# thanosDelatolas/eva-vos

Hardware: AMD Instinct MI355X
Metric: frames/sec STCN mask-propagate 480p 1-obj (higher is better)
Workload: dtype f32; 1 GPU; DAVIS-17-val-shaped 480x854 (padded 480x864) single-object STCN propagate: fresh engine, interact(mask,0), T=66 frames/video, mem_freq=5, top_k=50; one video per step per GPU; videos_per_gpu=38, streams_per_gpu=4, key_lookahead=0, clips=8 distinct synthetic clips (one per pooled engine), weights=synthetic recipe seed 0 (no checkpoints offline)

## Files before the change

eva_vos_amd/_lib.py:

```python
from __future__ import annotations

import ctypes as C
import os

import torch

_HERE = os.path.dirname(os.path.abspath(__file__))
LIB_PATH = os.environ.get("STCN_LIB") or os.path.join(_HERE, "libstcn_hip.so")

K_CLASSES = ("conv", "conv_reduce", "memread", "elementwise", "conv_n1", "other", "wino_input", "fusion_conv", "attention")


class WeightDesc(C.Structure):
    _fields_ = [("name", C.c_char_p), ("data", C.c_void_p), ("ndim", C.c_int32), ("shape", C.c_int64 * 4)]


class EngineOpts(C.Structure):
    _fields_ = [(n, C.c_int32) for n in ("lookahead", "decode_batch", "key_batch", "fuse_side")]


class ModelOpts(C.Structure):
    _fields_ = [("top_k", C.c_int32), ("km", C.c_float)]


# ... 22 lines not shown
    "stcn_test_transpose": (_I, [_P, _P, _P, _I, _I, _I, _L, _L, _I]),
    "stcn_engine_create": (_I, [_P, _I, _I, _I, _I, _I, _P, _P, _P, _P, C.POINTER(_P)]),
    "stcn_engine_create_ex": (_I, [_P, _I, _I, _I, _I, _I, _P, _P, _P, _P, C.POINTER(EngineOpts), C.POINTER(_P)]),
    "stcn_engine_get_opts": (_I, [_P, C.POINTER(EngineOpts)]),
    "stcn_engine_destroy": (_I, [_P]),
    "stcn_engine_reset": (_I, [_P]),
    "stcn_engine_clone": (_I, [_P, _P, _P, _P, C.POINTER(_P)]),
    "stcn_interact": (_I, [_P, _P, _I, _I, _I]),
    "stcn_get_stats": (_I, [_P, C.POINTER(Stats)]),
    "stcn_get_flops": (_I, [_P, C.POINTER(_D)]),
    "stcn_last_conv_path": (C.c_char_p, []),
    "stcn_test_conv_trace": (_I, [_I]),
    "stcn_test_conv_trace_get": (C.c_char_p, []),
    "stcn_test_conv": (_I, [_P, _P, _P, _P, _P, _P] + [_I] * 11),
    "stcn_test_conv_ex": (_I, [_P, _P, _P, _P, _P, _P] + [_I] * 11 + [_P, _I, _L, _L, _L, _I, _L]),
    "stcn_test_conv_path": (_I, [_I] * 9 + [C.c_char_p, _I]),
    "stcn_test_conv_plan": (_I, [_I] * 9 + [C.POINTER(C.c_int32), _I, C.POINTER(_D)]),
    "stcn_test_sweep_plan": (_I, [_I, _I, _I, _I, C.POINTER(C.c_int32), _I, C.POINTER(C.c_int32)]),
    "stcn_test_encode_key": (_I, [_P, _P, _P, _I, _I, _P, _P, _P, _P, _P]),
    "stcn_test_encode_value": (_I, [_P, _P, _P, _P, _P, _I, _I, _I, _P]),
    "stcn_test_memory_read": (_I, [_P, _P, _P, _P, _I, _I, _I, _P, _P, _P]),
    "stcn_test_memory_read_k": (_I, [_P, _P, _P, _P, _I, _I, _I, _I, _P, _P, _P]),
    "stcn_test_memory_read_km": (_I, [_P, _P, _P, _P, _I, _I, _I, _I, _I, _I, _F, _P, _P, _P, _P]),
    "stcn_bench_memory_read": (_I, [_P, _P, _P, _P, _I, _I, _I, _I, _P, C.POINTER(_F), C.POINTER(C.c_int32)]),
    "stcn_bench_memory_read_k": (_I, [_P, _P, _P, _P, _I, _I, _I, _I, _I, _P, C.POINTER(_F), C.POINTER(C.c_int32)]),
    "stcn_bench_memory_read_km": (_I, [_P, _P, _P, _P, _I, _I, _I, _I, _I, _I, _F, _I, _P, C.POINTER(_F), C.POINTER(C.c_int32)]),
    "stcn_memread_plan": (_I, [_I, _I, C.POINTER(C.c_int32)]),
    "stcn_memread_scratch": (_I, [_I, C.POINTER(C.c_int64)]),
    "stcn_test_kernel": (_I, [C.c_char_p, _P, C.POINTER(_P), _I, C.POINTER(C.c_int64), _I, C.POINTER(_D), _I]),
    "stcn_test_fail_at": (_I, [_I]),
    "stcn_test_side_delay_us": (_I, [_I]),
    "stcn_test_decode": (_I, [_P, _P, _P, _P, _P, _P, _I, _I, _I, _P, _P]),
    "stcn_test_attention": (_I, [_P, _P, _P, _P, _P, _I, _I, _I, _P]),
    "stcn_test_fusion": (_I, [_P, _P, _P, _P, _P, _P, _F, _F, _I, _I, _P]),
# ... 59 lines not shown
```

eva_vos_amd/csrc/conv_gemm.hip:

```cpp
#include <hip/hip_ext.h>

#include <cstdio>
#include <cstdlib>
#include <mutex>
#include <set>
#include <type_traits>
#include <utility>

#include "kernels.h"

namespace stcn {

typedef float f32x4 __attribute__((ext_vector_type(4)));
typedef float f32x16 __attribute__((ext_vector_type(16)));

static constexpr int BK = 32;
static constexpr int LDT = 36;

typedef unsigned u32x4 __attribute__((ext_vector_type(4)));
static constexpr unsigned OOB = 0x80000000u;

struct TileDiv { FastDiv ntile, tiles_n, per_panel; int tiles_m; };
__device__ __forceinline__ void tile_to_mn(int tile, int tiles_n, int ntile, int pn, const TileDiv &td, int &tm, int &tn) {
    if (pn > 0 && tiles_n % pn == 0 && tiles_n > pn) {
// ... 495 lines not shown
                __builtin_amdgcn_sched_barrier(0);
            }
        }
        __syncthreads();
        if (--k_left == 0) { k_left = nkt; tile_end(); }
    };
    const int total = ((tile1 - tile0 + tstep - 1) / tstep) * nkt;
    int it = 0;
    for (; it + 1 < total; it += 2) {
        step(I0{});
        step(I1{});
    }
    if (it < total) step(I0{});
}

static int pw_chain_tiles(const ConvP &p, int force_splitk) {
    if (!p.kn.pw_chain || force_splitk > 0 || !p.pointwise || !p.affine_out || p.N <= 32 || (p.Cin % 32) != 0) return 0;
    if ((p.N % 64) != 0 && ((long)p.M + 64) * p.N * 4 >= (1L << 31)) return 0;
    const long ntile = (long)((p.M + 63) / 64) * ((p.N + 63) / 64);
    const long resident = (long)device_cus() * STCN_PW_WAVES;
    if (ntile < resident + resident / 2) return 0;
    const long nt = (ntile + resident - 1) / resident;
    return (int)(nt > 16 ? 16 : nt);
}

__global__ __launch_bounds__(256) void conv_reduce_kernel(const ConvP p) {
    const long total4 = (long)p.M * p.N / 4;
    const int ohw = p.OH * p.OW;
    const long slab = (long)p.M * p.N;
    for (long i = blockIdx.x * 256L + threadIdx.x; i < total4; i += (long)gridDim.x * 256) {
// ... 99 lines not shown

void conv_plan(ConvP &p, int force_splitk, size_t ws_floats, ConvPlan &cp) {
    static const int big_mode = env_int("STCN_CONV_BIG", 1);
    Plan pl = plan_variant(p, false, force_splitk, ws_floats);
    constexpr int big_mink = 2304;
    const bool big_ok = big_mode != 0 && !narrow_variant(p) && !smallc_variant(p) && p.N >= 128 && p.Kp >= big_mink;
    if (big_ok) {
        const Plan pb = plan_variant(p, true, force_splitk, ws_floats);
        if (pb.cost < pl.cost || big_mode >= 2) pl = pb;
    }
    p.panel = 4;
    p.tile_big = pl.big; p.splitk = pl.splitk;
    p.rem_full = pl.rem_full; p.rem_split = pl.rem_split; p.rem_per = pl.rem_per;
    p.chain = pw_chain_tiles(p, force_splitk);
    if (p.chain) { p.tile_big = 0; p.splitk = 1; p.rem_full = p.rem_split = p.rem_per = 0; }
    static const bool dbg = getenv("STCN_CONV_PLAN_DEBUG") != nullptr;
    if (dbg)
        fprintf(stderr, "conv_plan M=%d N=%d K=%d: %s splitk=%d tail=(%d full, %d pieces of %d) cost %.0f\n", p.M, p.N, p.Kp,
                pl.big ? "128x128" : (narrow_variant(p) ? "128x32" : "64x64"), pl.splitk, pl.rem_full, pl.rem_split, pl.rem_per, pl.cost);
    cp.family = CONV_DIRECT;
    cp.variant = conv_variant_name(p);
    cp.splitk = p.splitk; cp.tail = p.rem_split > 1;
    cp.n_in = 0; cp.n_gemm = 1; cp.reduce = p.splitk > 1 || p.rem_split > 1;
    cp.fl_exec = cp.fl;
}

int device_cus() {
    static const int cus = [] { int dev = 0, n = 256; (void)hipGetDevice(&dev); (void)hipDeviceGetAttribute(&n, hipDeviceAttributeMultiprocessorCount, dev); return n > 0 ? n : 256; }();
    return cus;
}

void allow_big_lds(const void *kernel, size_t lds) {
    if (lds <= 64 * 1024) return;
    static std::mutex mu;
    static std::set<std::pair<int, const void *>> done;
    int dev = 0;
// ... 4 lines not shown
}

void conv_launch(const ConvP &p, hipStream_t s, hipEvent_t *ev_gemm, hipEvent_t *ev_red) {
    const bool narrow = narrow_variant(p), big = p.tile_big != 0;
    const int BM = narrow ? 128 : (big ? 128 : 64), BN = narrow ? 32 : (big ? 128 : 64);
    const int tiles_m = (p.M + BM - 1) / BM, tiles_n = (p.N + BN - 1) / BN;
    const int ntile = tiles_m * tiles_n;
    const int nkt = p.Kp / BK;
    const int per = (nkt + p.splitk - 1) / p.splitk;
    const size_t lds = (size_t)2 * (BM + BN) * LDT * sizeof(float);
    const bool tail = p.rem_split > 1;
    const dim3 grid(tail ? p.rem_full + (ntile - p.rem_full) * p.rem_split : ntile * p.splitk);
    const bool smallc = smallc_variant(p);
    const int pn = p.panel;
    const TileDiv td{fastdiv_make((unsigned)ntile), fastdiv_make((unsigned)tiles_n), fastdiv_make((unsigned)(tiles_m * (pn > 0 ? pn : 1))), tiles_m};
    if (p.chain) {
        const dim3 cgrid((unsigned)((ntile + p.chain - 1) / p.chain));
        launch(p.relu_in ? pw_chain_kernel<true> : pw_chain_kernel<false>, cgrid, dim3(256), lds, s, ev_gemm, p, tiles_n, ntile, p.chain, td);
        return;
    }
#define STCN_INST(WM_, WN_, RM_, RN_, SC_, RL_, ...) kfn = conv_gemm_kernel<WM_, WN_, RM_, RN_, SC_, RL_, ##__VA_ARGS__>
    auto STCN_INST(2, 2, 1, 1, false, false);
    const bool pw = p.pointwise && !big && !narrow && !smallc;
    const int key = (pw ? 16 : 0) | (big ? 8 : 0) | (narrow ? 4 : 0) | (smallc ? 2 : 0) | (p.relu_in ? 1 : 0);
    switch (key) {
        case 16: STCN_INST(2, 2, 1, 1, false, false, true); break;
        case 17: STCN_INST(2, 2, 1, 1, false, true, true); break;
        case 0: break;
        case 1: STCN_INST(2, 2, 1, 1, false, true); break;
        case 2: STCN_INST(2, 2, 1, 1, true, false); break;
// ... 147 lines not shown
```

eva_vos_amd/csrc/engine.cpp:

```cpp
#include "engine.h"
#include "src_hash.h"

#include <algorithm>
#include <atomic>
#include <cmath>
#include <cstdarg>
#include <cstdio>
#include <cstdlib>
#include <cstring>
#include <map>
#include <mutex>
#include <unordered_map>
#include <utility>

namespace stcn {

static thread_local char g_err[512] = "";
void set_error(const char *fmt, ...) {
    va_list ap;
    va_start(ap, fmt);
    vsnprintf(g_err, sizeof(g_err), fmt, ap);
    va_end(ap);
}
const char *get_error() { return g_err; }

Knobs Knobs::from_env() {
    Knobs k;
    k.wino_min_cin = env_int("STCN_WINO_MIN_CIN", k.wino_min_cin);
    k.wino_ppw = env_int("STCN_WINO_PPW", k.wino_ppw);
    k.wino4_chunk_mb = env_int("STCN_WINO4_CHUNK_MB", k.wino4_chunk_mb);
    k.fusion_conv12 = env_int("STCN_FUSION_CONV12", k.fusion_conv12) != 0;
    k.fusion_wino = env_int("STCN_FUSION_WINO", k.fusion_wino) != 0;
    k.pw_chain = env_int("STCN_PW_CHAIN", k.pw_chain);
    return k;
}

void Prof::reset() {
    for (int i = 0; i < STCN_K_COUNT; ++i) { flops[i] = 0; bytes[i] = 0; exec_flops[i] = 0; launches[i] = 0; }
    hbm_conv_flops = hbm_conv_bytes = hbm_conv_ms = 0; hbm_conv_launches = 0;
    wino2_flops = wino4_flops = 0;
    for (auto &e : events) { pool.push_back(e.a); pool.push_back(e.b); }
    events.clear();
}
Prof::Ev &Prof::push_pair(int cls, bool hbm) {
    Ev e; e.cls = cls; e.hbm = hbm;
    for (hipEvent_t *p : {&e.a, &e.b}) {
        if (!pool.empty()) { *p = pool.back(); pool.pop_back(); }
        else (void)hipEventCreate(p);
// ... 447 lines not shown
    p.relu_in = a.relu_in; p.relu_out = a.relu_out;
    p.fd_ohw = fastdiv_make((unsigned)(p.OH * p.OW));
    p.fd_ow = fastdiv_make((unsigned)p.OW);
    p.fd_cin = fastdiv_make((unsigned)p.Cin);
    p.fd_kw = fastdiv_make((unsigned)p.KW);
    p.pointwise = cw.kh == 1 && cw.kw == 1 && a.stride == 1 && !a.x1 && bs0 == (long)H * W * c0;
    p.affine_out = (a.y_bs == 0 || a.y_bs == (long)p.OH * p.OW * p.N) && (!a.res || (res_bs == (long)p.OH * p.OW * p.N && !a.res_bmod)) &&
                   ((long)p.M + 128) * p.N * 4 < (1L << 32);
    p.partial = w.splitk;
    p.kn = w.kn;
    pl = ConvPlan{};
    pl.fl = 2.0 * p.M * p.N * (double)(cw.kh * cw.kw * cw.cin);
    if (a.force_splitk <= 0 && (fusion_conv_plan(p, pl) || wino4_plan(p, m.wino4_min_wg, w.wino_v_floats, w.splitk_floats, pl) ||
                                wino_plan(p, w.wino_v_floats, w.splitk_floats, pl)))
        return STCN_OK;
    conv_plan(p, a.force_splitk, w.splitk_floats, pl);
    return STCN_OK;
}

int run_conv(const Model &m, Work &w, hipStream_t s, const std::string &name, const ConvArgs &a) {
    ConvP p;
    ConvPlan &pl = g_path.plan;
    const int rc = plan_conv(m, w, name, a, p, pl);
    if (rc) return rc;
    hipEvent_t *eg[W4_MAX_CHUNKS] = {}, *ei[W4_MAX_CHUNKS] = {}, *er = nullptr;
    if (w.prof) {
        const double in0 = (double)(p.bs0 ? p.B : 1) * p.H * p.W * p.c0, in1 = p.x1 ? (double)(p.bs1 ? p.B : 1) * p.H * p.W * p.c1 : 0.0;
        const double resb = p.res ? (p.res_bs ? (double)p.M * p.N : (double)p.OH * p.OW * p.N) : 0.0;
        const double bytes = 4.0 * (in0 + in1 + (double)p.N * p.K + (double)p.M * p.N + resb);
        const bool hbm_bound = pl.fl / bytes < 157.3e12 / 8.0e12;
        const int cls = w.conv_cls;
        const bool hbm_acc = hbm_bound && cls == STCN_K_CONV;
        w.prof->bytes[cls] += bytes;
        w.prof->flops[cls] += pl.fl;
        w.prof->exec_flops[cls] += pl.fl_exec;
        if (hbm_acc) { w.prof->hbm_conv_bytes += bytes; w.prof->hbm_conv_flops += pl.fl; }
        if (pl.family == CONV_WINO4) w.prof->wino4_flops += pl.fl; else if (pl.family == CONV_WINO2) w.prof->wino2_flops += pl.fl;
        for (int c = 0; c < pl.n_gemm; ++c) {
            eg[c] = w.prof->attach(cls, hbm_acc);
            if (c < pl.n_in) ei[c] = w.prof->attach(STCN_K_WINO_INPUT);
        }
        if (pl.reduce) er = w.prof->attach(STCN_K_CONV_REDUCE);
    }
    if (g_trace_on) { char b[96]; g_trace += name; g_trace += '='; g_trace += format_conv_path(pl, b, sizeof(b)); g_trace += '\n'; }
    switch (pl.family) {
    case CONV_FUSION: fusion_conv_launch(p, pl, s, eg[0]); break;
    case CONV_WINO4: wino4_launch(p, pl, w.wino_v, s, ei, eg, er); break;
    case CONV_WINO2: wino_launch(p, pl, w.wino_v, s, ei[0], eg[0], er); break;
    default: conv_launch(p, s, eg[0], er);
    }
    return launch_status(name.c_str());
}

#define RC(x) do { int rc_ = (x); if (rc_) return rc_; } while (0)

int encode_key(const Model &m, Work &w, hipStream_t s, const float *img4, const KeyOut &o, int B, long out_bs) {
    const Dims &d = w.d;
    const long obs = B > 1 ? out_bs : 0;
    const long ibs = obs ? obs : CONV_DENSE;
    RC(run_conv(m, w, s, "key_encoder.conv1", ConvArgs(img4, 4, B, d.nh, d.nw).strided(2).out(w.A).relu(0, 1)));
    { Scope sc(w.prof, STCN_K_ELEMWISE, s); maxpool3x3s2_launch(w.A, w.B, B, d.h2, d.w2, 64, s); }
    struct St { const char *name; int n, planes, stride; } stages[3] = {{"res2", 3, 64, 1}, {"layer2", 4, 128, 2}, {"layer3", 6, 256, 2}};
    int H = d.h4, W = d.w4, cin = 64;
    float *x = w.B;
    for (int si = 0; si < 3; ++si) {
        const St &st = stages[si];
        for (int i = 0; i < st.n; ++i) {
            const std::string p = std::string("key_encoder.") + st.name + "." + std::to_string(i);
            const int sd = i == 0 ? st.stride : 1;
            const int OH = H / sd, OW = W / sd;
            const float *idt = x;
            if (i == 0) { RC(run_conv(m, w, s, p + ".downsample.0", ConvArgs(x, cin, B, H, W).strided(sd).out(w.D))); idt = w.D; }
            RC(run_conv(m, w, s, p + ".conv1", ConvArgs(x, cin, B, H, W).out(w.C).relu(0, 1)));
            RC(run_conv(m, w, s, p + ".conv2", ConvArgs(w.C, st.planes, B, H, W).strided(sd).out(w.A).relu(0, 1)));
            float *dst = x;
            long dst_bs = 0;
            if (si == 2 && i == st.n - 1) { dst = o.f16; dst_bs = obs; }
            RC(run_conv(m, w, s, p + ".conv3", ConvArgs(w.A, st.planes, B, OH, OW).out(dst, dst_bs).residual(idt).relu(0, 1)));
            x = dst; H = OH; W = OW; cin = st.planes * 4;
        }
        if (si == 0) {
            if (o.f4_copy) HIPCHK(hipMemcpyAsync(o.f4_copy, x, (size_t)d.hw4 * 256 * 4, hipMemcpyDeviceToDevice, s));
            if (o.s4) RC(run_conv(m, w, s, "decoder.up_8_4.skip_conv", ConvArgs(x, 256, B, d.h4, d.w4).out(o.s4, obs)));
        } else if (si == 1) {
            if (o.f8_copy) HIPCHK(hipMemcpyAsync(o.f8_copy, x, (size_t)d.hw8 * 512 * 4, hipMemcpyDeviceToDevice, s));
            if (o.s8) RC(run_conv(m, w, s, "decoder.up_16_8.skip_conv", ConvArgs(x, 512, B, d.h8, d.w8).out(o.s8, obs)));
        }
    }
    if (o.k16) {
        RC(run_conv(m, w, s, "key_proj.key_proj", ConvArgs(o.f16, 1024, B, d.h16, d.w16, ibs).out(o.k16, obs)));
        if (o.msq) {
            Scope sc(w.prof, STCN_K_ELEMWISE, s);
            rowsumsq_launch(o.k16, d.hw16, 64, o.msq, s, B, out_bs, out_bs);
// ... 904 lines not shown
```

eva_vos_amd/csrc/engine.h:

```cpp
#pragma once
#include <hip/hip_runtime.h>

#include <deque>
#include <map>
#include <memory>
#include <set>
#include <string>
#include <vector>

#include "../../include/stcn_hip.h"
#include "kernels.h"

namespace stcn {

void set_error(const char *fmt, ...);
struct Model;
struct ConvW;
hipError_t pool_malloc(void **p, size_t bytes);
void pool_free(void *p);
void pool_release();
bool wants_wino(const ConvW &cw);
bool wants_wino4(const ConvW &cw);
bool wants_wino_fusion12(const ConvW &cw);
int make_wino(Model &m, ConvW &cw, const std::vector<float> &w_host);
// ... 93 lines not shown
void inject_failure_after(int n);
int launch_status(const char *what);
const char *last_conv_path();
void set_conv_path(const char *s);
void conv_trace(int on);
const char *conv_trace_get();
constexpr long CONV_DENSE = -1;
struct ConvArgs {
    const float *x0 = nullptr, *x1 = nullptr;
    int c0 = 0, c1 = 0;
    long bs0 = CONV_DENSE, bs1 = 0;
    int B = 1, H = 0, W = 0, stride = 1;
    float *y = nullptr; long y_bs = 0;
    const float *res = nullptr; long res_bs = CONV_DENSE; int res_bmod = 0;
    int relu_in = 0, relu_out = 0, force_splitk = 0;
    ConvArgs(const float *x, int c, int B_, int H_, int W_, long bs = CONV_DENSE) : x0(x), c0(c), bs0(bs), B(B_), H(H_), W(W_) {}
    ConvArgs &concat(const float *x, int c, long bs) { x1 = x; c1 = c; bs1 = bs; return *this; }
    ConvArgs &strided(int s) { stride = s; return *this; }
    ConvArgs &out(float *y_, long bs = 0) { y = y_; y_bs = bs; return *this; }
    ConvArgs &residual(const float *r, long bs = CONV_DENSE, int bmod = 0) { res = r; res_bs = bs; res_bmod = bmod; return *this; }
    ConvArgs &relu(int in, int out_) { relu_in = in; relu_out = out_; return *this; }
    ConvArgs &splitk(int k) { force_splitk = k; return *this; }
};
int plan_conv(const Model &m, const Work &w, const std::string &name, const ConvArgs &a, ConvP &p, ConvPlan &pl);
const char *format_conv_path(const ConvPlan &pl, char *out, size_t n);
int run_conv(const Model &m, Work &w, hipStream_t s, const std::string &name, const ConvArgs &a);
struct SweepGroup {
    int first;
    int t_lo;
    int G;
    bool inserts;
};
std::vector<SweepGroup> plan_sweep(int idx, int closest, int mem_freq, int cap);
constexpr int MAX_DECODE_GROUP = 8;
int encode_key(const Model &m, Work &w, hipStream_t s, const float *img4, const KeyOut &o, int B = 1, long out_bs = 0);
int encode_value(const Model &m, Work &w, hipStream_t s, const float *img4, const float *f16,
                 const float *masks, long mask_stride, float *out, long out_bs, const float *vd = nullptr,
// ... 61 lines not shown
```

eva_vos_amd/csrc/hooks.cpp:

```cpp
#include <algorithm>
#include <climits>
#include <cmath>
#include <cstdlib>
#include <cstring>
#include <string>
#include <vector>

#include "engine.h"

using namespace stcn;
#define RC(x) do { int rc_ = (x); if (rc_) return rc_; } while (0)

namespace {
struct TmpWork {
    Work w;
    int rc;
    TmpWork(int nh, int nw, int k) { rc = w.init(nh, nw, k); }
    ~TmpWork() { (void)hipDeviceSynchronize(); w.release(); }
};
struct DevBuf {
    float *p = nullptr;
    int alloc(size_t floats) { HIPCHK(hipMalloc((void **)&p, floats * 4)); return STCN_OK; }
    ~DevBuf() { if (p) { (void)hipDeviceSynchronize(); (void)hipFree(p); } }
};
ConvW test_convw(int Cin, int Cout, int KH, int KW) {
    ConvW cw;
    cw.cout = Cout; cw.cin = Cin; cw.cin_p = Cin; cw.kh = KH; cw.kw = KW;
    cw.K = KH * KW * Cin; cw.Kp = (cw.K + 31) / 32 * 32;
    return cw;
}
size_t test_wino_v_floats(int B, int OH, int OW, int Cin) {
    const size_t v2 = (size_t)16 * Cin * (((size_t)B * ((OH + 1) / 2) * ((OW + 1) / 2) + 63) / 64 * 64);
// ... 115 lines not shown
    }
    ConvRig r;
    RC(r.init(cw, wino ? &hw : nullptr, flags & 4, B, OH, OW, (size_t)16 * 1024 * 1024));
    if (wino && (flags & 4)) r.m.wino4_min_wg = 0;
    if (Cout == 1) {
        const bool dense = !x1 && bs0 == CONV_DENSE && y_bs == CONV_DENSE && !res;
        if (stride != 1 || !dense) { set_error("Cout==1 path is stride 1, one dense source, dense output, no residual"); return STCN_E_INVALID; }
        float b0 = 0.f;
        if (bias) HIPCHK(hipMemcpy(&b0, bias, 4, hipMemcpyDeviceToHost));
        conv_n1_launch(x, wpad.p, b0, y, B, H, W, Cin, KH, flags & 1, s);
        set_conv_path("n1");
    } else {
        RC(run_conv(r.m, r.w, s, "t", ConvArgs(x, Cin, B, H, W, bs0).concat(x1, c1, x1 ? bs1 : 0).strided(stride).out(y, y_bs == CONV_DENSE ? 0 : y_bs)
                                          .residual(res, res_bs, res_bmod).relu(flags & 1, (flags >> 1) & 1).splitk(splitk)));
    }
    HIPCHK(hipStreamSynchronize(s));
    HIPCHK(hipGetLastError());
    return STCN_OK;
}

int stcn_test_conv_path(int B, int H, int W, int Cin, int Cout, int K, int stride, int flags, int splitk, char *out, int n) {
    if (Cin % 4 || !out || n < 1) { set_error("stcn_test_conv_path: Cin%%4==0 and an output buffer required"); return STCN_E_INVALID; }
    ConvP p;
    ConvPlan pl;
    RC(plan_test_conv(B, H, W, Cin, Cout, K, stride, flags, splitk, p, pl));
    format_conv_path(pl, out, (size_t)n);
    return STCN_OK;
}

int stcn_test_conv_plan(int B, int H, int W, int Cin, int Cout, int K, int stride, int flags, int splitk, int32_t *iv, int n, double *dv) {
// ... 62 lines not shown
}

int stcn_test_encode_key(const stcn_model *m, void *stream, const float *img, int nh, int nw, float *k16, float *f16_thin,
                         float *f16, float *f8, float *f4) {
    if (!m || !img || nh % 16 || nw % 16) { set_error("stcn_test_encode_key: bad arguments"); return STCN_E_INVALID; }
    hipStream_t s = (hipStream_t)stream;
    TmpWork t(nh, nw, 1);
    RC(t.rc);
    const Dims &d = t.w.d;
    DevBuf img4, tf16, tk16, tmsq;
    RC(img4.alloc((size_t)d.npix * 4)); RC(tf16.alloc((size_t)d.hw16 * 1024)); RC(tk16.alloc((size_t)d.hw16 * 64));
    RC(tmsq.alloc(d.hw16));
    RC(pack_one(img, nh, nw, img4.p, s));
    KeyOut ko{k16 ? k16 : tk16.p, tmsq.p, f16_thin, f16 ? f16 : tf16.p, nullptr, nullptr, f8, f4, nullptr, nullptr};
    RC(encode_key(m->m, t.w, s, img4.p, ko));
    HIPCHK(hipStreamSynchronize(s));
    HIPCHK(hipGetLastError());
    return STCN_OK;
}

int stcn_test_encode_value(const stcn_model *m, void *stream, const float *img, const float *f16, const float *masks, int k,
                           int nh, int nw, float *out) {
    if (!m || !img || !f16 || !masks || !out || k < 1 || k > STCN_MAX_OBJECTS) { set_error("stcn_test_encode_value: bad arguments"); return STCN_E_INVALID; }
    hipStream_t s = (hipStream_t)stream;
    TmpWork t(nh, nw, k);
    RC(t.rc);
    DevBuf img4;
    RC(img4.alloc((size_t)t.w.d.npix * 4));
    RC(pack_one(img, nh, nw, img4.p, s));
    RC(encode_value(m->m, t.w, s, img4.p, f16, masks, t.w.d.npix, out, 0));
// ... 307 lines not shown
```

eva_vos_amd/csrc/kernels.h:

```cpp
#pragma once
#include <hip/hip_runtime.h>
#include <stdint.h>

#include <cstdlib>

#include "../../include/stcn_hip.h"

namespace stcn {

struct FastDiv {
    unsigned magic, shift, d;
};
static inline FastDiv fastdiv_make(unsigned d) {
    FastDiv f{0, 0, d};
    if (d <= 1) return f;
    unsigned s = 0;
    while ((1ull << s) < d) ++s;
    f.magic = (unsigned)(((1ull << (31 + s)) / d) + 1);
    f.shift = s - 1;
    return f;
}
#if defined(__HIPCC__)
__device__ __forceinline__ int fastdiv(int x, const FastDiv f) {
    return f.d <= 1 ? x : (int)(__umulhi((unsigned)x, f.magic) >> f.shift);
// ... 3 lines not shown
    return (xcd < r8 ? xcd * (q8 + 1) : r8 * (q8 + 1) + (xcd - r8) * q8) + (bid >> 3);
}
#endif

static inline int env_int(const char *name, int dflt) { const char *e = getenv(name); return e ? atoi(e) : dflt; }
static inline bool env_on(const char *name, bool dflt = true) { return env_int(name, dflt) != 0; }
int device_cus();

struct Knobs {
    int wino_min_cin = 128;
    int wino_ppw = 0;
    int wino4_chunk_mb = 160;
    int fusion_conv12 = 0;
    int fusion_wino = 1;
    int pw_chain = 2;
    static Knobs from_env();
};

struct ConvP {
    const float *x0, *x1;
    int c0, c1;
    long bs0, bs1;
    unsigned x0_bytes, x1_bytes, w_bytes;
    int B, H, W;
    int OH, OW;
    int KH, KW, stride, pad;
    int Cin;
    int M, N;
    int K, Kp;
    const float *w;
    const float *bias;
// ... 3 lines not shown
    float *y;
    long y_bs;
    int relu_in, relu_out;
    int splitk;
    float *partial;
    int rem_full, rem_split, rem_per;
    const float *wino_u;
    const float *wino4_u;
    FastDiv fd_ohw, fd_ow;
    FastDiv fd_cin, fd_kw;
    int pointwise;
    int affine_out;
    int tile_big;
    int panel;
    int chain;
    Knobs kn;
};
constexpr int W4_MAX_CHUNKS = 16;
struct WinoGeom { int TH, TW, Mt, Mt_pad, KB; };
struct W2Plan { int tiles_n, ntile, kb_per_split; };
struct W4Plan { int tiles_m, tiles_n, mb, grid, full_wg, pieces, per, chunks, tm_per_chunk, judge_wg; };
enum ConvFamily { CONV_LITERAL = 0, CONV_FUSION = 1, CONV_WINO4 = 2, CONV_WINO2 = 3, CONV_DIRECT = 4 };
struct ConvPlan {
    int family = CONV_LITERAL;
    bool fusion_wino = false;
    WinoGeom geo{};
    W4Plan w4{};
    W2Plan w2{};
    int splitk = 1;
    int ppw = 0;
// ... 115 lines not shown
```

include/stcn_hip.h:

```cpp
#ifndef STCN_HIP_H
#define STCN_HIP_H

#include <stddef.h>
#include <stdint.h>

#ifdef __cplusplus
extern "C" {
#endif

#define STCN_OK            0
#define STCN_E_INVALID    -1
#define STCN_E_MISSING    -2
#define STCN_E_HIP        -3
#define STCN_E_STATE      -4

#define STCN_MAX_OBJECTS  32

typedef struct stcn_model  stcn_model;
typedef struct stcn_engine stcn_engine;

typedef struct {
    const char  *name;
    const float *data;
    int32_t      ndim;
// ... 53 lines not shown
int stcn_stage_attention(stcn_stage *s, const float *mk16, const float *pos, const float *neg, const float *qk16, int b, float *attn);
int stcn_stage_fusion(stcn_stage *s, const float *im, const float *seg1, const float *seg2, const float *attn, float nc, float nr, float *logit);
int stcn_aggregate_wbg(void *stream, const float *prob, int k, long npix, int keep_bg, int hard, float *out);
int stcn_fusion_model_create(int device, const stcn_weight_desc *fuse, int n_fuse, stcn_model **out);
int stcn_test_transpose(void *stream, const float *src, float *dst, int B, int R, int C, long ld, long planes_bs, int to_rows);


int stcn_test_conv(void *stream, const float *x, const float *w, const float *bias, const float *res,
                   float *y, int B, int H, int W, int Cin, int Cout, int KH, int KW, int stride,
                   int pad, int flags, int splitk);

int stcn_test_conv_ex(void *stream, const float *x, const float *w, const float *bias, const float *res,
                      float *y, int B, int H, int W, int Cin, int Cout, int KH, int KW, int stride,
                      int pad, int flags, int splitk, const float *x1, int c1, long bs0, long bs1, long res_bs, int res_bmod, long y_bs);

int stcn_test_conv_path(int B, int H, int W, int Cin, int Cout, int K, int stride, int flags, int splitk, char *out, int n);
#define STCN_CONV_PLAN_INTS 27
int stcn_test_conv_plan(int B, int H, int W, int Cin, int Cout, int K, int stride, int flags, int splitk, int32_t *iv, int n, double *dv);
const char *stcn_last_conv_path(void);
int stcn_test_sweep_plan(int idx, int closest, int mem_freq, int cap, int32_t *out, int n, int32_t *count);
int stcn_test_conv_trace(int on);
const char *stcn_test_conv_trace_get(void);

int stcn_test_kernel(const char *name, void *stream, void *const *ptrs, int nptr, const int64_t *iv, int ni, const double *fv, int nf);

int stcn_test_encode_key(const stcn_model *m, void *stream, const float *img, int nh, int nw,
                         float *k16, float *f16_thin, float *f16, float *f8, float *f4);

int stcn_test_encode_value(const stcn_model *m, void *stream, const float *img, const float *f16,
                           const float *masks, int k, int nh, int nw, float *out);

int stcn_test_memory_read(void *stream, const float *mk, const float *mv, const float *qk,
                          int N, int Q, int k, int32_t *topk_idx, float *topk_w, float *readout);
int stcn_test_memory_read_k(void *stream, const float *mk, const float *mv, const float *qk,
                            int N, int Q, int k, int top_k, int32_t *topk_idx, float *topk_w, float *readout);
int stcn_test_memory_read_km(void *stream, const float *mk, const float *mv, const float *qk,
                             int N, int Q, int k, int top_k, int h16, int w16, float km, int32_t *centres,
                             int32_t *topk_idx, float *topk_w, float *readout);

int stcn_bench_memory_read(void *stream, const float *mk, const float *mv, const float *qk, int N, int Q, int k,
                           int iters, float *readout, float *ms, int32_t *plan7);
int stcn_bench_memory_read_k(void *stream, const float *mk, const float *mv, const float *qk, int N, int Q, int k, int top_k,
// ... 59 lines not shown
```

Measured before the change: 833.6 frames/s.

## Fuse consecutive pointwise convs in ResNet res2 blocks into one pair kernel

```diff
diff --git a/eva_vos_amd/_lib.py b/eva_vos_amd/_lib.py
--- a/eva_vos_amd/_lib.py
+++ b/eva_vos_amd/_lib.py
@@ -60,10 +60,12 @@
     "stcn_test_conv_trace_get": (C.c_char_p, []),
     "stcn_test_conv": (_I, [_P, _P, _P, _P, _P, _P] + [_I] * 11),
     "stcn_test_conv_ex": (_I, [_P, _P, _P, _P, _P, _P] + [_I] * 11 + [_P, _I, _L, _L, _L, _I, _L]),
+    "stcn_test_conv_pair": (_I, [_P] * 11 + [_I] * 7 + [_L, C.c_char_p, _I]),
     "stcn_test_conv_path": (_I, [_I] * 9 + [C.c_char_p, _I]),
     "stcn_test_conv_plan": (_I, [_I] * 9 + [C.POINTER(C.c_int32), _I, C.POINTER(_D)]),
     "stcn_test_sweep_plan": (_I, [_I, _I, _I, _I, C.POINTER(C.c_int32), _I, C.POINTER(C.c_int32)]),
     "stcn_test_encode_key": (_I, [_P, _P, _P, _I, _I, _P, _P, _P, _P, _P]),
+    "stcn_test_encode_key_batch": (_I, [_P, _P, _P, _I, _I, _I, _P, _L, C.POINTER(C.c_int64)]),
     "stcn_test_encode_value": (_I, [_P, _P, _P, _P, _P, _I, _I, _I, _P]),
     "stcn_test_memory_read": (_I, [_P, _P, _P, _P, _I, _I, _I, _P, _P, _P]),
     "stcn_test_memory_read_k": (_I, [_P, _P, _P, _P, _I, _I, _I, _I, _P, _P, _P]),
diff --git a/eva_vos_amd/csrc/conv_gemm.hip b/eva_vos_amd/csrc/conv_gemm.hip
--- a/eva_vos_amd/csrc/conv_gemm.hip
+++ b/eva_vos_amd/csrc/conv_gemm.hip
@@ -533,6 +533,256 @@
     if (it < total) step(I0{});
 }
 
+#ifndef STCN_PAIR_WG64
+#define STCN_PAIR_WG64 2
+#endif
+template <int RN2>
+__global__ __launch_bounds__(256, RN2 == 1 ? STCN_PAIR_WG64 : 2) void pw_pair_kernel(const ConvP p) {
+    constexpr int BM = 64, N1 = 256, TS = 68, NB = 2 * RN2, N2 = 64 * RN2;
+    extern __shared__ __attribute__((aligned(16))) float smem[];
+    float *As = smem;
+    float *Bs = As + 2 * BM * LDT;
+    float *T = Bs + 2 * N2 * LDT;
+    const int nb = gridDim.x, swz = xcd_contiguous_block((int)blockIdx.x, nb);
+    const int tiles_m = (p.M + BM - 1) / BM;
+    if (swz >= tiles_m) return;
+    const int t = threadIdx.x, lane = t & 63, wave = t >> 6;
+    const int wm = wave >> 1, wn = wave & 1;
+    const int kc = t & 7, r0 = t >> 3;
+    const int prow = t >> 4, pseg = t & 15;
+    const int nkt1 = p.Kp / BK;
+    const unsigned y1_bytes = (unsigned)((long)p.M * N1 * 4), y2_bytes = (unsigned)((long)p.M * N2 * 4);
+    const __amdgpu_buffer_rsrc_t rs0 = __builtin_amdgcn_make_buffer_rsrc(const_cast<float *>(p.x0), 0, p.x0_bytes, 0x00020000);
+    const __amdgpu_buffer_rsrc_t rsw1 = __builtin_amdgcn_make_buffer_rsrc(const_cast<float *>(p.w), 0, p.w_bytes, 0x00020000);
+    const __amdgpu_buffer_rsrc_t rsw2 = __builtin_amdgcn_make_buffer_rsrc(const_cast<float *>(p.pair.w2), 0, (unsigned)(N2 * N1 * 4), 0x00020000);
+    const __amdgpu_buffer_rsrc_t ry1 = __builtin_amdgcn_make_buffer_rsrc(p.y, 0, y1_bytes, 0x00020000);
+    const __amdgpu_buffer_rsrc_t rr = __builtin_amdgcn_make_buffer_rsrc(const_cast<float *>(p.res ? p.res : p.y), 0, y1_bytes, 0x00020000);
+    const __amdgpu_buffer_rsrc_t ry2 = __builtin_amdgcn_make_buffer_rsrc(p.pair.y2, 0, y2_bytes, 0x00020000);
+
+    unsigned aoff[2];
+    bool l_live = true;
+    int l_tile = swz, l_tn = 0, l_pos = 0;
+    auto set_load_tile = [&](int tile) {
+        l_live = tile < tiles_m;
+#pragma unroll
+        for (int i = 0; i < 2; ++i) {
+            const int m = tile * BM + r0 + 32 * i;
+            aoff[i] = l_live && m < p.M ? (unsigned)((m * p.c0 + kc * 4) * 4) : OOB;
+        }
+    };
+    set_load_tile(swz);
+    f32x4 ra[2][2], rb[2][NB];
+    unsigned va[2], vb[NB];
+    bool g_p1 = true;
+    auto g_step = [&]() {
+        g_p1 = l_pos < nkt1;
+        const unsigned k1 = (unsigned)l_pos * (BK * 4u), k2 = (unsigned)(l_tn * 2 + l_pos - nkt1) * (BK * 4u);
+#pragma unroll
+        for (int i = 0; i < 2; ++i) va[i] = g_p1 ? aoff[i] + k1 : OOB;
+#pragma unroll
+        for (int i = 0; i < NB; ++i) {
+            const unsigned w1 = i < 2 ? (unsigned)(((l_tn * 64 + r0 + 32 * i) * p.Kp + kc * 4) * 4) + k1 : OOB;
+            const unsigned w2 = (unsigned)(((r0 + 32 * i) * N1 + kc * 4) * 4) + k2;
+            vb[i] = l_live ? (g_p1 ? w1 : w2) : OOB;
+        }
+        if (++l_pos == nkt1 + 2) {
+            l_pos = 0;
+            if (++l_tn == 4) { l_tn = 0; l_tile += nb; set_load_tile(l_tile); }
+        }
+    };
+    auto g_a = [&](int i, auto setc) {
+        constexpr int ST = decltype(setc)::value;
+        ra[ST][i] = __builtin_bit_cast(f32x4, __builtin_amdgcn_raw_buffer_load_b128(rs0, va[i], 0, 0));
+    };
+    auto g_b = [&](int i, auto setc) {
+        constexpr int ST = decltype(setc)::value;
+        rb[ST][i] = __builtin_bit_cast(f32x4, __builtin_amdgcn_raw_buffer_load_b128(g_p1 ? rsw1 : rsw2, vb[i], 0, 0));
+    };
+    float *const a_st = As + r0 * LDT + kc * 4;
+    float *const b_st = Bs + r0 * LDT + kc * 4;
+    auto s_a = [&](int i, int buf, auto setc) {
+        constexpr int ST = decltype(setc)::value;
+        *reinterpret_cast<f32x4 *>(a_st + (buf * BM + 32 * i) * LDT) = ra[ST][i];
+    };
+    auto s_b = [&](int i, int buf, auto setc) {
+        constexpr int ST = decltype(setc)::value;
+        *reinterpret_cast<f32x4 *>(b_st + (buf * N2 + 32 * i) * LDT) = rb[ST][i];
+    };
+    using I0 = std::integral_constant<int, 0>;
+    using I1 = std::integral_constant<int, 1>;
+    auto gload_all = [&](auto setc) {
+        g_step();
+#pragma unroll
+        for (int i = 0; i < 2; ++i) g_a(i, setc);
+#pragma unroll
+        for (int i = 0; i < NB; ++i) g_b(i, setc);
+    };
+    constexpr int NL = 2 + NB;
+    auto staging = [&](int slot, int ns, int buf, auto gsc) {
+        constexpr int GS = decltype(gsc)::value;
+        using SS = std::integral_constant<int, GS ^ 1>;
+        if (slot == 0) g_step();
+        else if (slot <= 2) g_a(slot - 1, gsc);
+        else if (slot <= NL) g_b(slot - 3, gsc);
+        else if (slot >= ns - 1 - NL && slot < ns - 1 - NB) s_a(slot - (ns - 1 - NL), buf ^ 1, SS{});
+        else if (slot >= ns - 1 - NB && slot < ns - 1) s_b(slot - (ns - 1 - NB), buf ^ 1, SS{});
+    };
+
+    f32x16 acc1, acc2[RN2], part2[RN2];
+#pragma unroll
+    for (int i = 0; i < 16; ++i) acc1[i] = 0.f;
+#pragma unroll
+    for (int b = 0; b < RN2; ++b)
+#pragma unroll
+        for (int i = 0; i < 16; ++i) { acc2[b][i] = 0.f; part2[b][i] = 0.f; }
+    const bool split2 = p.pair.split2 != 0;
+    const int arow = (wm * 32 + (lane & 31)) * LDT + (lane >> 5) * 4;
+    const int brow = (wn * 32 + (lane & 31)) * LDT + (lane >> 5) * 4;
+    const int trow = (wm * 32 + (lane & 31)) * TS + (lane >> 5) * 4;
+    auto step1 = [&](auto gsc) {
+        constexpr int buf = decltype(gsc)::value;
+        const float *a_s = As + buf * BM * LDT + arow;
+        const float *b_s = Bs + buf * N2 * LDT + brow;
+        f32x4 fa[2], fb[2];
+        fa[0] = *reinterpret_cast<const f32x4 *>(a_s);
+        fb[0] = *reinterpret_cast<const f32x4 *>(b_s);
+#pragma unroll
+        for (int kb = 0; kb < 4; ++kb) {
+            const int cur = kb & 1;
+            if (kb < 3) {
+                fa[cur ^ 1] = *reinterpret_cast<const f32x4 *>(a_s + (kb + 1) * 8);
+                fb[cur ^ 1] = *reinterpret_cast<const f32x4 *>(b_s + (kb + 1) * 8);
+            }
+#pragma unroll
+            for (int j = 0; j < 4; ++j) {
+                acc1 = __builtin_amdgcn_mfma_f32_32x32x2f32(fa[cur][j], fb[cur][j], acc1, 0, 0, 0);
+                staging(4 * kb + j, 16, buf, gsc);
+                __builtin_amdgcn_sched_barrier(0);
+            }
+        }
+        __syncthreads();
+    };
+    auto step2 = [&](auto gsc, int kt2) {
+        constexpr int buf = decltype(gsc)::value;
+        const float *a_s = T + trow + kt2 * BK;
+        const float *b_s = Bs + buf * N2 * LDT + brow;
+        f32x4 fa[2], fb[2][RN2];
+        fa[0] = *reinterpret_cast<const f32x4 *>(a_s);
+#pragma unroll
+        for (int b = 0; b < RN2; ++b) fb[0][b] = *reinterpret_cast<const f32x4 *>(b_s + b * 64 * LDT);
+#pragma unroll
+        for (int kb = 0; kb < 4; ++kb) {
+            const int cur = kb & 1;
+            if (kb < 3) {
+                fa[cur ^ 1] = *reinterpret_cast<const f32x4 *>(a_s + (kb + 1) * 8);
+#pragma unroll
+                for (int b = 0; b < RN2; ++b) fb[cur ^ 1][b] = *reinterpret_cast<const f32x4 *>(b_s + b * 64 * LDT + (kb + 1) * 8);
+            }
+#pragma unroll
+            for (int j = 0; j < 4; ++j)
+#pragma unroll
+                for (int b = 0; b < RN2; ++b) {
+                    acc2[b] = __builtin_amdgcn_mfma_f32_32x32x2f32(fa[cur][j], fb[cur][b][j], acc2[b], 0, 0, 0);
+                    staging((4 * kb + j) * RN2 + b, 16 * RN2, buf, gsc);
+                    __builtin_amdgcn_sched_barrier(0);
+                }
+        }
+        __syncthreads();
+    };
+
+    float *const t_acc = T + (wm * 32 + 4 * (lane >> 5)) * TS + wn * 32 + (lane & 31);
+    float *const t_pc = T + prow * TS + pseg * 4;
+    const float lo1 = p.relu_out ? 0.f : -__builtin_inff(), lo2 = p.pair.relu2 ? 0.f : -__builtin_inff();
+    float bv2[RN2];
+#pragma unroll
+    for (int b = 0; b < RN2; ++b) bv2[b] = p.pair.bias2 ? p.pair.bias2[b * 64 + wn * 32 + (lane & 31)] : 0.f;
+    f32x4 rres[4];
+    float bv1 = 0.f;
+    auto slice_begin = [&](int tile, int tn) {
+        bv1 = p.bias ? p.bias[tn * 64 + wn * 32 + (lane & 31)] : 0.f;
+        const unsigned o0 = p.res ? ((unsigned)(tile * BM + prow) * N1 + (unsigned)(tn * 64 + pseg * 4)) * 4u : OOB;
+#pragma unroll
+        for (int i = 0; i < 4; ++i)
+            rres[i] = __builtin_bit_cast(f32x4, __builtin_amdgcn_raw_buffer_load_b128(rr, o0 + (unsigned)(16 * i * N1 * 4), 0, 0));
+    };
+    auto slice_end = [&](int tile, int tn) {
+#pragma unroll
+        for (int r = 0; r < 16; ++r) t_acc[((r & 3) + 8 * (r >> 2)) * TS] = acc1[r] + bv1;
+#pragma unroll
+        for (int i = 0; i < 16; ++i) acc1[i] = 0.f;
+        __syncthreads();
+        const unsigned o0 = ((unsigned)(tile * BM + prow) * N1 + (unsigned)(tn * 64 + pseg * 4)) * 4u;
+        f32x4 v[4];
+#pragma unroll
+        for (int i = 0; i < 4; ++i) v[i] = *reinterpret_cast<const f32x4 *>(t_pc + 16 * i * TS);
+#pragma unroll
+        for (int i = 0; i < 4; ++i) {
+            v[i].x = fmaxf(v[i].x + rres[i].x, lo1); v[i].y = fmaxf(v[i].y + rres[i].y, lo1);
+            v[i].z = fmaxf(v[i].z + rres[i].z, lo1); v[i].w = fmaxf(v[i].w + rres[i].w, lo1);
+        }
+#pragma unroll
+        for (int i = 0; i < 4; ++i) {
+            *reinterpret_cast<f32x4 *>(t_pc + 16 * i * TS) = v[i];
+            __builtin_amdgcn_raw_buffer_store_b128(__builtin_bit_cast(u32x4, v[i]), ry1, o0 + (unsigned)(16 * i * N1 * 4), 0, 0);
+        }
+        __syncthreads();
+    };
+    auto tile_end = [&](int tile) {
+#pragma unroll
+        for (int b = 0; b < RN2; ++b) {
+#pragma unroll
+            for (int r = 0; r < 16; ++r)
+                t_acc[((r & 3) + 8 * (r >> 2)) * TS] = fmaxf(split2 ? (part2[b][r] + acc2[b][r]) + bv2[b] : acc2[b][r] + bv2[b] + 0.f, lo2);
+#pragma unroll
+            for (int i = 0; i < 16; ++i) acc2[b][i] = 0.f;
+            __syncthreads();
+            const unsigned o0 = ((unsigned)(tile * BM + prow) * N2 + (unsigned)(b * 64 + pseg * 4)) * 4u;
+#pragma unroll
+            for (int i = 0; i < 4; ++i) {
+                const f32x4 v = *reinterpret_cast<const f32x4 *>(t_pc + 16 * i * TS);
+                __builtin_amdgcn_raw_buffer_store_b128(__builtin_bit_cast(u32x4, v), ry2, o0 + (unsigned)(16 * i * N2 * 4), 0, 0);
+            }
+            __syncthreads();
+        }
+    };
+
+    gload_all(I0{});
+    gload_all(I1{});
+    s_a(0, 0, I0{}); s_a(1, 0, I0{});
+#pragma unroll
+    for (int i = 0; i < NB; ++i) s_b(i, 0, I0{});
+    __syncthreads();
+    for (int tile = swz; tile < tiles_m; tile += nb) {
+        for (int tn = 0; tn < 4; ++tn) {
+            slice_begin(tile, tn);
+            for (int kt = 0; kt < nkt1; kt += 2) {
+                step1(I0{});
+                step1(I1{});
+            }
+            slice_end(tile, tn);
+            step2(I0{}, 0);
+            step2(I1{}, 1);
+            if (split2 && tn == 1) {
+#pragma unroll
+                for (int b = 0; b < RN2; ++b) {
+                    part2[b] = acc2[b];
+#pragma unroll
+                    for (int i = 0; i < 16; ++i) acc2[b][i] = 0.f;
+                }
+            }
+        }
+        tile_end(tile);
+    }
+}
+
+static int pw_pair_tiles(const ConvP &p, int force_splitk) {
+    const int N2 = p.pair.N2;
+    if (!p.kn.pw_pair || force_splitk > 0 || !p.pointwise || !p.affine_out || p.relu_in || p.N != 256 || (N2 != 64 && N2 != 128)) return 0;
+    if ((p.Cin % 64) != 0 || p.Kp != p.Cin) return 0;
+    const long tiles_m = (p.M + 63) / 64, resident = (long)device_cus() * (N2 == 64 ? STCN_PAIR_WG64 : 2);
+    return (int)((tiles_m + resident - 1) / resident);
+}
+
 static int pw_chain_tiles(const ConvP &p, int force_splitk) {
     if (!p.kn.pw_chain || force_splitk > 0 || !p.pointwise || !p.affine_out || p.N <= 32 || (p.Cin % 32) != 0) return 0;
     if ((p.N % 64) != 0 && ((long)p.M + 64) * p.N * 4 >= (1L << 31)) return 0;
@@ -662,12 +912,26 @@
     p.rem_full = pl.rem_full; p.rem_split = pl.rem_split; p.rem_per = pl.rem_per;
     p.chain = pw_chain_tiles(p, force_splitk);
     if (p.chain) { p.tile_big = 0; p.splitk = 1; p.rem_full = p.rem_split = p.rem_per = 0; }
+    if (p.pair.N2) {
+        p.pair.tiles = pw_pair_tiles(p, force_splitk);
+        if (p.pair.tiles) {
+            ConvP p2 = p;
+            p2.Cin = p2.K = p2.Kp = p.N; p2.c0 = p.N; p2.N = p.pair.N2; p2.res = nullptr; p2.pair = PwPair{};
+            const Plan pl2 = plan_variant(p2, false, 0, ws_floats);
+            const bool unsplit = pw_chain_tiles(p2, 0) > 0 || (pl2.splitk == 1 && pl2.rem_split <= 1);
+            p.pair.split2 = !unsplit && pl2.splitk == 2 && pl2.rem_split <= 1;
+            if (!unsplit && !p.pair.split2) p.pair.tiles = 0;
+        }
+        if (p.pair.tiles) { p.chain = 0; p.tile_big = 0; p.splitk = 1; p.rem_full = p.rem_split = p.rem_per = 0; }
+        else p.pair = PwPair{};
+    }
     static const bool dbg = getenv("STCN_CONV_PLAN_DEBUG") != nullptr;
     if (dbg)
         fprintf(stderr, "conv_plan M=%d N=%d K=%d: %s splitk=%d tail=(%d full, %d pieces of %d) cost %.0f\n", p.M, p.N, p.Kp,
                 pl.big ? "128x128" : (narrow_variant(p) ? "128x32" : "64x64"), pl.splitk, pl.rem_full, pl.rem_split, pl.rem_per, pl.cost);
     cp.family = CONV_DIRECT;
-    cp.variant = conv_variant_name(p);
+    cp.variant = p.pair.N2 ? (p.pair.N2 == 64 ? "pw_pair N2=64" : "pw_pair N2=128") : conv_variant_name(p);
+    if (p.pair.N2) cp.fl += 2.0 * p.M * p.pair.N2 * (double)p.N;
     cp.splitk = p.splitk; cp.tail = p.rem_split > 1;
     cp.n_in = 0; cp.n_gemm = 1; cp.reduce = p.splitk > 1 || p.rem_split > 1;
     cp.fl_exec = cp.fl;
@@ -702,6 +966,13 @@
     const bool smallc = smallc_variant(p);
     const int pn = p.panel;
     const TileDiv td{fastdiv_make((unsigned)ntile), fastdiv_make((unsigned)tiles_n), fastdiv_make((unsigned)(tiles_m * (pn > 0 ? pn : 1))), tiles_m};
+    if (p.pair.N2) {
+        const int tm64 = (p.M + 63) / 64, rn2 = p.pair.N2 / 64;
+        const dim3 pgrid((unsigned)((tm64 + p.pair.tiles - 1) / p.pair.tiles));
+        const size_t plds = (size_t)(2 * 64 * LDT + 2 * 64 * rn2 * LDT + 64 * 68) * sizeof(float);
+        launch(rn2 == 1 ? pw_pair_kernel<1> : pw_pair_kernel<2>, pgrid, dim3(256), plds, s, ev_gemm, p);
+        return;
+    }
     if (p.chain) {
         const dim3 cgrid((unsigned)((ntile + p.chain - 1) / p.chain));
         launch(p.relu_in ? pw_chain_kernel<true> : pw_chain_kernel<false>, cgrid, dim3(256), lds, s, ev_gemm, p, tiles_n, ntile, p.chain, td);
diff --git a/eva_vos_amd/csrc/engine.cpp b/eva_vos_amd/csrc/engine.cpp
--- a/eva_vos_amd/csrc/engine.cpp
+++ b/eva_vos_amd/csrc/engine.cpp
@@ -32,6 +32,7 @@
     k.fusion_conv12 = env_int("STCN_FUSION_CONV12", k.fusion_conv12) != 0;
     k.fusion_wino = env_int("STCN_FUSION_WINO", k.fusion_wino) != 0;
     k.pw_chain = env_int("STCN_PW_CHAIN", k.pw_chain);
+    k.pw_pair = env_int("STCN_PW_PAIR", k.pw_pair) != 0;
     return k;
 }
 
@@ -509,6 +510,13 @@
     if (a.force_splitk <= 0 && (fusion_conv_plan(p, pl) || wino4_plan(p, m.wino4_min_wg, w.wino_v_floats, w.splitk_floats, pl) ||
                                 wino_plan(p, w.wino_v_floats, w.splitk_floats, pl)))
         return STCN_OK;
+    if (!a.pair_name.empty()) {
+        auto i2 = m.conv.find(a.pair_name);
+        if (i2 == m.conv.end()) { set_error("missing conv '%s'", a.pair_name.c_str()); return STCN_E_MISSING; }
+        const ConvW &c2 = i2->second;
+        if (c2.cin_p != cw.cout) { set_error("conv '%s': %d input channels, '%s' gives %d", a.pair_name.c_str(), c2.cin_p, name.c_str(), cw.cout); return STCN_E_INVALID; }
+        if (c2.kh == 1 && c2.kw == 1 && c2.Kp == c2.cin_p) p.pair = PwPair{c2.w, c2.bias, a.pair_y, c2.cout, a.pair_relu, 0, 0};
+    }
     conv_plan(p, a.force_splitk, w.splitk_floats, pl);
     return STCN_OK;
 }
@@ -522,7 +530,8 @@
     if (w.prof) {
         const double in0 = (double)(p.bs0 ? p.B : 1) * p.H * p.W * p.c0, in1 = p.x1 ? (double)(p.bs1 ? p.B : 1) * p.H * p.W * p.c1 : 0.0;
         const double resb = p.res ? (p.res_bs ? (double)p.M * p.N : (double)p.OH * p.OW * p.N) : 0.0;
-        const double bytes = 4.0 * (in0 + in1 + (double)p.N * p.K + (double)p.M * p.N + resb);
+        const double pairb = p.pair.N2 ? (double)p.pair.N2 * p.N + (double)p.M * p.pair.N2 : 0.0;
+        const double bytes = 4.0 * (in0 + in1 + (double)p.N * p.K + (double)p.M * p.N + resb + pairb);
         const bool hbm_bound = pl.fl / bytes < 157.3e12 / 8.0e12;
         const int cls = w.conv_cls;
         const bool hbm_acc = hbm_bound && cls == STCN_K_CONV;
@@ -544,7 +553,9 @@
     case CONV_WINO2: wino_launch(p, pl, w.wino_v, s, ei[0], eg[0], er); break;
     default: conv_launch(p, s, eg[0], er);
     }
-    return launch_status(name.c_str());
+    const int st = launch_status(name.c_str());
+    if (st || a.pair_name.empty() || p.pair.N2) return st;
+    return run_conv(m, w, s, a.pair_name, ConvArgs(a.y, p.N, p.B, p.OH, p.OW, a.y_bs ? a.y_bs : CONV_DENSE).out(a.pair_y).relu(0, a.pair_relu));
 }
 
 #define RC(x) do { int rc_ = (x); if (rc_) return rc_; } while (0)
@@ -558,6 +569,7 @@
     struct St { const char *name; int n, planes, stride; } stages[3] = {{"res2", 3, 64, 1}, {"layer2", 4, 128, 2}, {"layer3", 6, 256, 2}};
     int H = d.h4, W = d.w4, cin = 64;
     float *x = w.B;
+    bool c1_done = false;
     for (int si = 0; si < 3; ++si) {
         const St &st = stages[si];
         for (int i = 0; i < st.n; ++i) {
@@ -566,12 +578,15 @@
             const int OH = H / sd, OW = W / sd;
             const float *idt = x;
             if (i == 0) { RC(run_conv(m, w, s, p + ".downsample.0", ConvArgs(x, cin, B, H, W).strided(sd).out(w.D))); idt = w.D; }
-            RC(run_conv(m, w, s, p + ".conv1", ConvArgs(x, cin, B, H, W).out(w.C).relu(0, 1)));
+            if (!c1_done) RC(run_conv(m, w, s, p + ".conv1", ConvArgs(x, cin, B, H, W).out(w.C).relu(0, 1)));
             RC(run_conv(m, w, s, p + ".conv2", ConvArgs(w.C, st.planes, B, H, W).strided(sd).out(w.A).relu(0, 1)));
             float *dst = x;
             long dst_bs = 0;
             if (si == 2 && i == st.n - 1) { dst = o.f16; dst_bs = obs; }
-            RC(run_conv(m, w, s, p + ".conv3", ConvArgs(w.A, st.planes, B, OH, OW).out(dst, dst_bs).residual(idt).relu(0, 1)));
+            ConvArgs c3 = ConvArgs(w.A, st.planes, B, OH, OW).out(dst, dst_bs).residual(idt).relu(0, 1);
+            c1_done = si == 0 && w.kn.pw_pair;
+            if (c1_done) c3.pair(i + 1 < st.n ? std::string("key_encoder.res2.") + std::to_string(i + 1) + ".conv1" : std::string("key_encoder.layer2.0.conv1"), w.C, 1);
+            RC(run_conv(m, w, s, p + ".conv3", c3));
             x = dst; H = OH; W = OW; cin = st.planes * 4;
         }
         if (si == 0) {
diff --git a/eva_vos_amd/csrc/engine.h b/eva_vos_amd/csrc/engine.h
--- a/eva_vos_amd/csrc/engine.h
+++ b/eva_vos_amd/csrc/engine.h
@@ -131,6 +131,7 @@
     float *y = nullptr; long y_bs = 0;
     const float *res = nullptr; long res_bs = CONV_DENSE; int res_bmod = 0;
     int relu_in = 0, relu_out = 0, force_splitk = 0;
+    std::string pair_name; float *pair_y = nullptr; int pair_relu = 0;
     ConvArgs(const float *x, int c, int B_, int H_, int W_, long bs = CONV_DENSE) : x0(x), c0(c), bs0(bs), B(B_), H(H_), W(W_) {}
     ConvArgs &concat(const float *x, int c, long bs) { x1 = x; c1 = c; bs1 = bs; return *this; }
     ConvArgs &strided(int s) { stride = s; return *this; }
@@ -138,6 +139,7 @@
     ConvArgs &residual(const float *r, long bs = CONV_DENSE, int bmod = 0) { res = r; res_bs = bs; res_bmod = bmod; return *this; }
     ConvArgs &relu(int in, int out_) { relu_in = in; relu_out = out_; return *this; }
     ConvArgs &splitk(int k) { force_splitk = k; return *this; }
+    ConvArgs &pair(const std::string &name, float *y2, int relu_out2) { pair_name = name; pair_y = y2; pair_relu = relu_out2; return *this; }
 };
 int plan_conv(const Model &m, const Work &w, const std::string &name, const ConvArgs &a, ConvP &p, ConvPlan &pl);
 const char *format_conv_path(const ConvPlan &pl, char *out, size_t n);
diff --git a/eva_vos_amd/csrc/hooks.cpp b/eva_vos_amd/csrc/hooks.cpp
--- a/eva_vos_amd/csrc/hooks.cpp
+++ b/eva_vos_amd/csrc/hooks.cpp
@@ -15,7 +15,7 @@
 struct TmpWork {
     Work w;
     int rc;
-    TmpWork(int nh, int nw, int k) { rc = w.init(nh, nw, k); }
+    TmpWork(int nh, int nw, int k, int key_batch = 1) { rc = w.init(nh, nw, k, key_batch); }
     ~TmpWork() { (void)hipDeviceSynchronize(); w.release(); }
 };
 struct DevBuf {
@@ -161,6 +161,32 @@
         RC(run_conv(r.m, r.w, s, "t", ConvArgs(x, Cin, B, H, W, bs0).concat(x1, c1, x1 ? bs1 : 0).strided(stride).out(y, y_bs == CONV_DENSE ? 0 : y_bs)
                                           .residual(res, res_bs, res_bmod).relu(flags & 1, (flags >> 1) & 1).splitk(splitk)));
     }
+    HIPCHK(hipStreamSynchronize(s));
+    HIPCHK(hipGetLastError());
+    return STCN_OK;
+}
+
+int stcn_test_conv_pair(void *stream, const float *x, const float *w1, const float *b1, const float *res, const float *w2, const float *b2,
+                        float *y1, float *y2, float *y1_ref, float *y2_ref, int B, int H, int W, int K1, int N1, int N2, int flags, long y_bs,
+                        char *path, int n) {
+    if (!x || !w1 || !w2 || !y1 || !y2 || !y1_ref || !y2_ref || B < 1 || H < 1 || W < 1 || K1 < 32 || K1 % 32 || N1 < 32 || N1 % 32 || N2 < 1 ||
+        y_bs < CONV_DENSE || (path && n < 1)) {
+        set_error("stcn_test_conv_pair: all tensors but bias / res, B, H, W, N2 >= 1, K1 and N1 multiples of 32, y_bs -1 (dense) or elements required");
+        return STCN_E_INVALID;
+    }
+    hipStream_t s = (hipStream_t)stream;
+    ConvW c1 = test_convw(K1, N1, 1, 1), c2 = test_convw(N1, N2, 1, 1);
+    c1.w = const_cast<float *>(w1); c1.bias = const_cast<float *>(b1);
+    c2.w = const_cast<float *>(w2); c2.bias = const_cast<float *>(b2);
+    ConvRig r;
+    RC(r.init(c1, nullptr, false, B, H, W, (size_t)16 * 1024 * 1024));
+    r.m.conv["t2"] = c2;
+    const int relu1 = flags & 1, relu2 = (flags >> 1) & 1;
+    const long ybs = y_bs == CONV_DENSE ? 0 : y_bs;
+    RC(run_conv(r.m, r.w, s, "t", ConvArgs(x, K1, B, H, W).out(y1, ybs).residual(res).relu(0, relu1).pair("t2", y2, relu2)));
+    if (path) snprintf(path, (size_t)n, "%s", last_conv_path());
+    RC(run_conv(r.m, r.w, s, "t", ConvArgs(x, K1, B, H, W).out(y1_ref, ybs).residual(res).relu(0, relu1).splitk(1)));
+    RC(run_conv(r.m, r.w, s, "t2", ConvArgs(y1_ref, N1, B, H, W, ybs ? ybs : CONV_DENSE).out(y2_ref).relu(0, relu2)));
     HIPCHK(hipStreamSynchronize(s));
     HIPCHK(hipGetLastError());
     return STCN_OK;
@@ -253,6 +279,36 @@
     RC(pack_one(img, nh, nw, img4.p, s));
     KeyOut ko{k16 ? k16 : tk16.p, tmsq.p, f16_thin, f16 ? f16 : tf16.p, nullptr, nullptr, f8, f4, nullptr, nullptr};
     RC(encode_key(m->m, t.w, s, img4.p, ko));
+    HIPCHK(hipStreamSynchronize(s));
+    HIPCHK(hipGetLastError());
+    return STCN_OK;
+}
+
+int stcn_test_encode_key_batch(const stcn_model *m, void *stream, const float *imgs, int B, int nh, int nw, float *out, long slot, int64_t *offsets) {
+    if (!m || !imgs || !offsets || B < 1 || nh < 16 || nw < 16 || nh % 16 || nw % 16) { set_error("stcn_test_encode_key_batch: bad arguments"); return STCN_E_INVALID; }
+    hipStream_t s = (hipStream_t)stream;
+    Dims d;
+    d.set(nh, nw);
+    const char *names[4] = {"decoder.up_16_8.skip_conv", "decoder.up_8_4.skip_conv", "decoder.compress.downsample#b", "decoder.compress.conv1#b"};
+    long c[4];
+    for (int i = 0; i < 4; ++i) {
+        auto it = m->m.conv.find(names[i]);
+        if (it == m->m.conv.end()) { set_error("stcn_test_encode_key_batch: missing conv '%s'", names[i]); return STCN_E_MISSING; }
+        c[i] = it->second.cout;
+    }
+    const long sizes[8] = {(long)d.hw16 * 64, (long)d.hw16 + 64, (long)d.hw16 * 512, (long)d.hw16 * 1024, d.hw8 * c[0], d.hw4 * c[1], d.hw16 * c[2], d.hw16 * c[3]};
+    long off[9] = {0};
+    for (int i = 0; i < 8; ++i) { offsets[i] = off[i]; off[i + 1] = off[i] + (sizes[i] + 3) / 4 * 4; }
+    offsets[8] = off[8];
+    if (!out) return STCN_OK;
+    if (slot < off[8]) { set_error("stcn_test_encode_key_batch: a slot holds %ld floats, %ld given", off[8], slot); return STCN_E_INVALID; }
+    TmpWork t(nh, nw, 1, B);
+    RC(t.rc);
+    DevBuf img4;
+    RC(img4.alloc((size_t)B * d.npix * 4));
+    for (int b = 0; b < B; ++b) RC(pack_one(imgs + (size_t)b * 3 * d.npix, nh, nw, img4.p + (size_t)b * d.npix * 4, s));
+    KeyOut ko{out + off[0], out + off[1], out + off[2], out + off[3], out + off[4], out + off[5], nullptr, nullptr, out + off[6], out + off[7]};
+    RC(encode_key(m->m, t.w, s, img4.p, ko, B, slot));
     HIPCHK(hipStreamSynchronize(s));
     HIPCHK(hipGetLastError());
     return STCN_OK;
diff --git a/eva_vos_amd/csrc/kernels.h b/eva_vos_amd/csrc/kernels.h
--- a/eva_vos_amd/csrc/kernels.h
+++ b/eva_vos_amd/csrc/kernels.h
@@ -41,7 +41,16 @@
     int fusion_conv12 = 0;
     int fusion_wino = 1;
     int pw_chain = 2;
+    int pw_pair = 1;
     static Knobs from_env();
+};
+
+struct PwPair {
+    const float *w2;
+    const float *bias2;
+    float *y2;
+    int N2, relu2, tiles;
+    int split2;
 };
 
 struct ConvP {
@@ -75,6 +84,7 @@
     int tile_big;
     int panel;
     int chain;
+    PwPair pair;
     Knobs kn;
 };
 constexpr int W4_MAX_CHUNKS = 16;
diff --git a/include/stcn_hip.h b/include/stcn_hip.h
--- a/include/stcn_hip.h
+++ b/include/stcn_hip.h
@@ -91,6 +91,10 @@
                       float *y, int B, int H, int W, int Cin, int Cout, int KH, int KW, int stride,
                       int pad, int flags, int splitk, const float *x1, int c1, long bs0, long bs1, long res_bs, int res_bmod, long y_bs);
 
+int stcn_test_conv_pair(void *stream, const float *x, const float *w1, const float *b1, const float *res, const float *w2, const float *b2,
+                        float *y1, float *y2, float *y1_ref, float *y2_ref, int B, int H, int W, int K1, int N1, int N2, int flags, long y_bs,
+                        char *path, int n);
+
 int stcn_test_conv_path(int B, int H, int W, int Cin, int Cout, int K, int stride, int flags, int splitk, char *out, int n);
 #define STCN_CONV_PLAN_INTS 27
 int stcn_test_conv_plan(int B, int H, int W, int Cin, int Cout, int K, int stride, int flags, int splitk, int32_t *iv, int n, double *dv);
@@ -103,6 +107,8 @@
 
 int stcn_test_encode_key(const stcn_model *m, void *stream, const float *img, int nh, int nw,
                          float *k16, float *f16_thin, float *f16, float *f8, float *f4);
+
+int stcn_test_encode_key_batch(const stcn_model *m, void *stream, const float *imgs, int B, int nh, int nw, float *out, long slot, int64_t *offsets);
 
 int stcn_test_encode_value(const stcn_model *m, void *stream, const float *img, const float *f16,
                            const float *masks, int k, int nh, int nw, float *out);
```

Result: no change. 831.4 frames/s (-0.3%).
